# DixianZhu/deBWT

Hardware: AMD Instinct MI355X
Metric: Gbp/sec BWT build (30 Gbp synthetic DNA); bit-exact vs CPU ref; 1/2/4/8-GPU (higher is better)
Workload: dtype u64

## Files before the change

debwt_amd/_lib.py:

```python
import ctypes
import os
import subprocess

_HERE = os.path.dirname(os.path.abspath(__file__))
LIB_PATH = os.environ.get("DEBWT_HIP_LIB", os.path.join(_HERE, "libdebwt_hip.so"))
_lib = None


class DebwtConfig(ctypes.Structure):
    _fields_ = [("k", ctypes.c_int), ("device", ctypes.c_int), ("sort_algo", ctypes.c_int),
                ("reserved", ctypes.c_int)]


class DebwtPackedText(ctypes.Structure):
    _fields_ = [("words", ctypes.POINTER(ctypes.c_uint64)), ("nwords", ctypes.c_uint64), ("n", ctypes.c_uint64),
                ("sep", ctypes.POINTER(ctypes.c_uint64)), ("nrec", ctypes.c_uint64),
                ("seconds_read", ctypes.c_double), ("seconds_pack", ctypes.c_double)]


class DebwtStats(ctypes.Structure):
    _fields_ = ([(n, ctypes.c_uint64) for n in (
        "n", "nrec", "red_capacity", "blue_capacity", "blue_bound_num", "case3num", "sp_len",
        "special_branch_num", "n_main", "distinct_keys", "blue_large_blocks", "blue_max_block")] +
        [(n, ctypes.c_float) for n in (
# ... 231 lines not shown


class DebwtFmMapStats(ctypes.Structure):
    _fields_ = ([(n, ctypes.c_uint64) for n in ("reads", "mapped", "mems", "seeds", "candidates", "jobs", "batches")] +
                [(n, ctypes.c_float) for n in ("ms_mems", "ms_locate", "ms_candidates", "ms_extend", "ms_wall")])

    def as_dict(self):
        return {n: getattr(self, n) for n, _ in self._fields_}


class DebwtMultiStats(ctypes.Structure):
    _fields_ = [("n", ctypes.c_uint64), ("nrec", ctypes.c_uint64), ("ngpus", ctypes.c_uint32), ("rounds", ctypes.c_uint32),
                ("key_bytes_in", ctypes.c_uint64), ("blue_bytes_in", ctypes.c_uint64), ("ms_build", ctypes.c_float),
                ("key_mode", ctypes.c_uint32), ("exchange_backend", ctypes.c_uint32)]

    def as_dict(self):
        return {n: getattr(self, n) for n, _ in self._fields_}


SYMBOLS = [
    "debwt_create", "debwt_destroy", "debwt_strerror", "debwt_last_error", "debwt_load_text",
    "debwt_load_ascii", "debwt_kmer_sort_rle", "debwt_classify", "debwt_sp_generate", "debwt_blue_sort",
    "debwt_bwt_assemble", "debwt_build", "debwt_fetch_bwt", "debwt_bwt_device_ptr", "debwt_get_stats",
    "debwt_fetch_array", "debwt_kmer_count_sorted", "debwt_radix_sort_u64", "debwt_radix_sort_u64_range", "debwt_radix_pair_passes", "debwt_radix_bucket_passes", "debwt_verify_inverse",
    "debwt_shard_begin", "debwt_shard_histogram", "debwt_shard_set_range", "debwt_shard_classify_local",
    "debwt_shard_facts_export", "debwt_shard_classify_global", "debwt_shard_info", "debwt_shard_fetch",
    "debwt_shard_partition_keys", "debwt_shard_plan", "debwt_shard_ranges", "debwt_shard_sort_begin",
    "debwt_shard_sort_range", "debwt_shard_sort_end", "debwt_concat_rows", "debwt_shard_export", "debwt_census_words", "debwt_shard_sp_flags", "debwt_shard_sp_emit",
    "debwt_shard_sp_import", "debwt_shard_blue_route", "debwt_shard_blue_place", "debwt_set_range_cap", "debwt_pack_fasta", "debwt_free_packed", "debwt_load_fasta", "debwt_pack_fasta_opts", "debwt_load_fasta_opts", "debwt_fasta_text_bound", "debwt_host_release_hold", "debwt_special_digest", "debwt_bwt_census", "debwt_fetch_rows", "debwt_verify_device", "debwt_multi_create", "debwt_multi_destroy", "debwt_multi_last_error",
    "debwt_multi_load_text", "debwt_multi_load_fasta", "debwt_multi_build", "debwt_multi_fetch_bwt", "debwt_multi_get_stats",
    "debwt_multi_verify", "debwt_multi_shard", "debwt_pinned_alloc", "debwt_pinned_free", "debwt_shard_key_mode",
    "debwt_multi_set_key_mode", "debwt_special_compare", "debwt_build_to_host", "debwt_multi_set_exchange", "debwt_reserve",
    "debwt_multi_set_serial", "debwt_multi_get_shard_report", "debwt_multi_step_name", "debwt_get_config",
    "debwt_dump_reference_files", "debwt_shard_scratch",
    "debwt_fm_create", "debwt_fm_open", "debwt_fm_last_error", "debwt_fm_info_get", "debwt_fm_samples",
    "debwt_fm_record_starts", "debwt_fm_count", "debwt_fm_locate", "debwt_fm_destroy",
    "debwt_fm_search", "debwt_fm_search_stats_get", "debwt_fm_mems", "debwt_fm_mems_stats_get",
    "debwt_fm_attach_text", "debwt_fm_extend", "debwt_fm_extend_stats_get", "debwt_fm_cluster_seeds",
    "debwt_fm_map_defaults", "debwt_fm_map", "debwt_fm_map_stats_get",
    "debwt_fm_chain_seeds", "debwt_fm_extend_chain", "debwt_fm_chain_defaults", "debwt_fm_map_chained",
    "debwt_fm_align_window", "debwt_fm_insert_bounds", "debwt_fm_pair_select", "debwt_fm_pair_defaults",
    "debwt_fm_map_pairs", "debwt_fm_pair_stats_get",
    "debwt_fm_overlaps", "debwt_fm_overlaps_stats_get", "debwt_fm_overlap_longest",
    "debwt_fm_overlaps_mm", "debwt_fm_overlaps_mm_stats_get",
    "debwt_fm_extract", "debwt_fm_extract_stats_get", "debwt_fm_restore_text", "debwt_fm_text_fetch",
    "debwt_fm_kmer_counts", "debwt_fm_kmer_stats_get", "debwt_fm_weak_trials", "debwt_fm_correct_defaults",
    "debwt_fm_correct", "debwt_fm_correct_stats_get",
# ... 39 lines not shown
        fn = getattr(L, name)
        fn.restype = ctypes.c_int
        fn.argtypes = [vp]
    L.debwt_fetch_bwt.restype = ctypes.c_int
    L.debwt_fetch_bwt.argtypes = [vp, u64p, u64p, u64p]
    L.debwt_reserve.restype = ctypes.c_int
    L.debwt_reserve.argtypes = [vp, ctypes.c_uint64, ctypes.c_uint64, ctypes.c_double, ctypes.c_uint]
    L.debwt_build_to_host.restype = ctypes.c_int
    L.debwt_build_to_host.argtypes = [vp, u64p, u64p, u64p]
    L.debwt_bwt_device_ptr.restype = ctypes.c_int
    L.debwt_bwt_device_ptr.argtypes = [vp, ctypes.POINTER(vp)]
    L.debwt_get_stats.restype = ctypes.c_int
    L.debwt_get_stats.argtypes = [vp, ctypes.POINTER(DebwtStats)]
    L.debwt_fetch_array.restype = ctypes.c_int
    L.debwt_fetch_array.argtypes = [vp, ctypes.c_int, vp, ctypes.c_uint64, u64p]
    L.debwt_kmer_count_sorted.restype = ctypes.c_int
    L.debwt_kmer_count_sorted.argtypes = [vp, u64p, u64p, ctypes.c_uint64, u64p]
    L.debwt_radix_sort_u64.restype = ctypes.c_int
    L.debwt_radix_sort_u64.argtypes = [vp, vp, vp, ctypes.c_uint64, ctypes.c_int, ctypes.POINTER(ctypes.c_float)]
    L.debwt_radix_pair_passes.restype = ctypes.c_uint64
    L.debwt_radix_pair_passes.argtypes = []
    L.debwt_radix_bucket_passes.restype = ctypes.c_uint64
    L.debwt_radix_bucket_passes.argtypes = []
    L.debwt_radix_sort_u64_range.restype = ctypes.c_int
    L.debwt_radix_sort_u64_range.argtypes = [vp, vp, vp, ctypes.c_uint64, ctypes.c_int, ctypes.c_uint64, ctypes.c_uint64,
                                             ctypes.POINTER(ctypes.c_float)]
    L.debwt_verify_inverse.restype = ctypes.c_int
    L.debwt_verify_inverse.argtypes = [u64p, ctypes.c_uint64, u64p, ctypes.c_uint64, ctypes.c_uint64,
                                       ctypes.POINTER(ctypes.c_uint8)]
    L.debwt_shard_begin.restype = ctypes.c_int
    L.debwt_shard_begin.argtypes = [vp, ctypes.c_int, ctypes.c_int]
    L.debwt_shard_histogram.restype = ctypes.c_int
    L.debwt_shard_histogram.argtypes = [vp, u64p]
    L.debwt_shard_set_range.restype = ctypes.c_int
    L.debwt_shard_set_range.argtypes = [vp, ctypes.c_uint32, ctypes.c_uint32, ctypes.c_uint64, ctypes.c_uint64]
    L.debwt_shard_classify_local.restype = ctypes.c_int
    L.debwt_shard_classify_local.argtypes = [vp, u64p, u64p, u64p]
    L.debwt_shard_facts_export.restype = ctypes.c_int
    L.debwt_shard_facts_export.argtypes = [vp, vp, ctypes.c_uint64]
    L.debwt_shard_classify_global.restype = ctypes.c_int
    L.debwt_shard_classify_global.argtypes = [vp, vp, ctypes.c_uint64, ctypes.c_uint64, ctypes.c_uint64]
    u8p, u32p = ctypes.POINTER(ctypes.c_uint8), ctypes.POINTER(ctypes.c_uint32)
    L.debwt_shard_partition_keys.restype = ctypes.c_int
    L.debwt_shard_partition_keys.argtypes = [vp, u8p, vp, ctypes.c_uint64, u64p]
    L.debwt_shard_plan.restype = ctypes.c_int
    L.debwt_shard_plan.argtypes = [vp, u64p, ctypes.c_uint32, ctypes.c_uint32, ctypes.c_uint64, ctypes.c_int,
# ... 214 lines not shown
```

debwt_amd/csrc/debwt_hip.hip:

```cpp
#include "../../include/debwt_hip.h"

#include <hip/hip_runtime.h>

#include <algorithm>
#include <new>
#include <chrono>
#include <cmath>
#include <cstdio>
#include <cstring>
#include <atomic>
#include <string>
#include <thread>
#include <tuple>
#include <vector>

#include "radix_sort.h"
#include "special_host.h"
#include "fasta_host.h"
#include "gz_parallel.h"
#include "stage_kernels.h"
#include "special_kernels.h"
#include "verify_kernels.h"
#include "fm_kernels.h"
#include "fm_search_kernels.h"
// ... 2336 lines not shown
    KmerInfoF f{sorted, Mk, k, c->dk.as<u64>(), c->dstart.as<u32>()};
    if ((rc = cp_count(c, f, Mk, cp_area(c, 0), 0))) return rc;
    if ((rc = cp_emit(c, f, Mk, cp_area(c, 0)))) return rc;
    if ((rc = sync_check(c))) return rc;
    u64 D = c->h_scalars[0];
    *distinct = D;
    u64 ncopy = std::min<u64>(D, capacity);
    if (kmers && ncopy) HIPCHK(c, hipMemcpy(kmers, c->dk.p, ncopy * 8, hipMemcpyDeviceToHost));
    if (counts && ncopy) {
        std::vector<u32> first(D);
        HIPCHK(c, hipMemcpy(first.data(), c->dstart.p, D * 4, hipMemcpyDeviceToHost));
        for (u64 i = 0; i < ncopy; i++) counts[i] = (i + 1 < D ? first[i + 1] : (u32)Mk) - first[i];
    }
    return DEBWT_OK;
}

extern "C" int debwt_radix_sort_u64(debwt_ctx *c, uint64_t *d_keys, uint64_t *d_tmp, uint64_t count, int key_bits,
                                    float *ms_per_pass) {
    return debwt_radix_sort_u64_range(c, d_keys, d_tmp, count, key_bits, 0, 0, ms_per_pass);
}

extern "C" uint64_t debwt_radix_pair_passes(void) { return radix_pair_passes(); }
extern "C" uint64_t debwt_radix_bucket_passes(void) { return radix_bucket_passes(); }

__global__ void k_keys_outside(const u64 *__restrict__ keys, u64 n, u64 lo, u64 hi, u32 *__restrict__ flag) {
    bool bad = false;
    for (u64 i = (u64)blockIdx.x * blockDim.x + threadIdx.x; i < n; i += (u64)gridDim.x * blockDim.x) bad |= keys[i] < lo || keys[i] > hi;
    if (bad) *flag = 1u;
}

extern "C" int debwt_radix_sort_u64_range(debwt_ctx *c, uint64_t *d_keys, uint64_t *d_tmp, uint64_t count, int key_bits,
                                          uint64_t key_lo, uint64_t key_hi, float *ms_per_pass) {
    if (!c || !d_keys || !d_tmp || key_bits < 1 || key_bits > 64) return DEBWT_EINVAL;
    if (key_hi && key_hi <= key_lo) return DEBWT_EINVAL;
    if (count >= 0xFFFFFFF0ull) return DEBWT_ERANGE;
    HIPCHK(c, hipSetDevice(c->cfg.device));
    ENSURE(c, c->rs_skew, (count / 2048 + 2) * 4);
    ENSURE(c, c->rs_over, radix_over_bytes(count));
    const u64 range[2] = {key_lo, key_hi};
    const u64 *rg = key_lo || key_hi ? range : nullptr;
    if (rg) {
        const u64 top = key_bits >= 64 ? ~0ull : (1ull << key_bits) - 1ull;
        u32 outside = 0;
        HIPCHK(c, hipMemsetAsync(c->rs_over.p, 0, 4, c->stream));
        k_keys_outside<<<(u32)std::min<u64>(2048, (count + 255) / 256), 256, 0, c->stream>>>((const u64 *)d_keys, count, key_lo, key_hi ? key_hi - 1 : top,
                                                                                            c->rs_over.as<u32>());
// ... 3626 lines not shown
```

debwt_amd/csrc/radix_sort.h:

```cpp
#pragma once
#include "common.h"

#define RS_BLOCK 256
#ifndef RS_ITEMS
#define RS_ITEMS 16
#endif
#define RS_TILE (RS_BLOCK * RS_ITEMS)
#ifndef RS_MAXCHUNKS
#define RS_MAXCHUNKS 16384
#endif
#define RS_MINCHUNKS 2048
#ifndef RS_CHUNK_TILES
#define RS_CHUNK_TILES 64
#endif
#define RS_RADIX 256

struct RadixWorkspace {
    u32 *counts;
    u32 *over;
    u32 *h_over;
    u32 over_cap;
    u32 *skew_list;
    u32 *pair;
    size_t pair_cap;
};

size_t radix_pair_bytes(u64 n, int lo_bit, int hi_bit, bool aux, const u64 *range);
size_t radix_pair_bytes_u64(u64 n, int key_bits, const u64 *range, bool heavy = false);
u64 radix_pair_passes();

struct RadixSplit { bool hybrid, bucket; int T, pshift, hbm_shift; };
RadixSplit radix_split(u64 n, int key_bits, int algo, const u64 *range, bool heavy);
u64 radix_bucket_passes();
#define RS_BUCKET_HEAVY (1u << 20)

struct TextKeySrc {
    const u64 *text;
    const u64 *sepbits;
    u64 n;
    int K;
    u64 key_lo, key_hi;
    u64 pos0;
    const u32 *pre_counts;
    const u8 *bin_tab;
    int bin_shift;
};

#define RS_MAX_RANGES 16
size_t radix_text_hist_stride();
hipError_t radix_text_hist_ranges(hipStream_t stream, const TextKeySrc &text, const u8 *range_of_bin, int key_bits,
                                  const int *shift, int nranges, u32 *counts);

struct RsDigit {
    int shift; u32 mask;
    int mode;
    const u8 *tab; int tshift;
// ... 30 lines not shown
```

debwt_amd/csrc/radix_sort.hip:

```cpp
#include "radix_sort.h"

#include <algorithm>
#include <atomic>
#include <cstddef>
#include <utility>
#include <cstdio>
#include <cstdlib>
#include <vector>


template <int FIXED0>
__device__ __forceinline__ u32 rs_digit(const RsDigit &g, u64 k) {
    if (FIXED0 == 2) return __builtin_amdgcn_ubfe((u32)(k >> 32), (u32)g.shift - 32u, (u32)__popc(g.mask));
    if (FIXED0 || g.mode == 0) {
        const u32 lo = (u32)k, hi = (u32)(k >> 32);
        const bool up = g.shift >= 32;
        return __builtin_amdgcn_alignbit(up ? 0u : hi, up ? hi : lo, (u32)g.shift & 31u) & g.mask;
    }
    if (g.mode == 1) return g.tab[(k >> g.tshift) & 4095u];
    u32 q = (u32)(k >> g.tshift), lo = 0, hi = g.nb;
    if (hi <= 16u) {
        for (u32 i = 1; i < hi; i++) lo += g.bounds[i] <= q ? 1u : 0u;
        return lo;
    }
// ... 950 lines not shown
    const u64 p = keys[x - 1] >> pshift;
    for (u64 base = x; base < x + reach; base += 64) {
        u64 i = base + lane;
        bool diff = i >= n || (keys[i] >> pshift) != p;
        u64 mk = __ballot(diff);
        if (mk) return base + (u64)__ffsll((long long)mk) - 1;
    }
    u64 lo = x + reach, hi = n;
    while (lo < hi) {
        u64 mid = (lo + hi) >> 1;
        if ((keys[mid] >> pshift) <= p) lo = mid + 1; else hi = mid;
    }
    return lo;
}

#define RL_PAD(x) ((x) + ((x) >> 4))

__device__ __forceinline__ void rl_cex(u64 &a, u64 &b, bool up) {
    bool sw = (a > b) == up;
    u64 lo = sw ? b : a, hi = sw ? a : b;
    a = lo; b = hi;
}

__device__ __forceinline__ void rl_sort16(u64 (&k)[16]) {
#define RL_CE(a, b) rl_cex(k[a], k[b], true)
    RL_CE(0, 13); RL_CE(1, 12); RL_CE(2, 15); RL_CE(3, 14); RL_CE(4, 8); RL_CE(5, 6); RL_CE(7, 11); RL_CE(9, 10);
    RL_CE(0, 5); RL_CE(1, 7); RL_CE(2, 9); RL_CE(3, 4); RL_CE(6, 13); RL_CE(8, 14); RL_CE(10, 15); RL_CE(11, 12);
    RL_CE(0, 1); RL_CE(2, 3); RL_CE(4, 5); RL_CE(6, 8); RL_CE(7, 9); RL_CE(10, 11); RL_CE(12, 13); RL_CE(14, 15);
    RL_CE(0, 2); RL_CE(1, 3); RL_CE(4, 10); RL_CE(5, 11); RL_CE(6, 7); RL_CE(8, 9); RL_CE(12, 14); RL_CE(13, 15);
    RL_CE(1, 2); RL_CE(3, 12); RL_CE(4, 6); RL_CE(5, 7); RL_CE(8, 10); RL_CE(9, 11); RL_CE(13, 14);
    RL_CE(1, 4); RL_CE(2, 6); RL_CE(5, 8); RL_CE(7, 10); RL_CE(9, 13); RL_CE(11, 14);
    RL_CE(2, 4); RL_CE(3, 6); RL_CE(9, 12); RL_CE(11, 13);
    RL_CE(3, 5); RL_CE(6, 8); RL_CE(7, 9); RL_CE(10, 12);
    RL_CE(3, 4); RL_CE(5, 6); RL_CE(7, 8); RL_CE(9, 10); RL_CE(11, 12);
    RL_CE(6, 7); RL_CE(8, 9);
#undef RL_CE
}

template <int LG>
__device__ __forceinline__ void rl_network(u64 (&k)[16], u64 *A, const u32 tid, const bool active) {
    constexpr int KPT = 16;
#pragma unroll
    for (int lk = 1; lk <= LG; lk++) {
        const u32 kk = 1u << lk;
#pragma unroll
        for (int lj = lk - 1; lj >= 0; lj--) {
            if (lj < 4) {
                const int jj = 1 << lj;
// ... 19 lines not shown
                const u32 dt = 1u << (lj - 4);
                if (active) {
#pragma unroll
                    for (int r = 0; r < KPT; r++) A[RL_PAD(tid * KPT + r)] = k[r];
                }
                __syncthreads();
                const bool lower = (tid & dt) == 0;
                if (active) {
#pragma unroll
                    for (int r = 0; r < KPT; r++) {
                        u64 pk = A[RL_PAD((tid ^ dt) * KPT + r)];
                        bool up = ((tid * KPT + r) & kk) == 0;
                        bool take_min = lower == up;
                        bool pless = pk < k[r];
                        k[r] = (take_min == pless) ? pk : k[r];
                    }
                }
                __syncthreads();
            }
        }
    }
}

template <int NT>
__global__ __launch_bounds__(NT) void rs_local_kernel(u64 *__restrict__ keys, u64 n, int pshift,
                                                       u32 *__restrict__ over, u32 over_cap, u8 *__restrict__ mark) {
    constexpr int KPT = 16;
    constexpr u32 CAP = NT * KPT;
    constexpr u32 H = NT == 64 ? RLW_H : RL_H;
    constexpr int LOGN = NT == 64 ? 10 : 12;
    static_assert(NT == 64 || NT == 256, "wave or 4-wave workgroup");
    __shared__ u64 A[CAP + CAP / 16];
    __shared__ u64 sb[2];
    const u32 tid = threadIdx.x;
    if (NT == 256 && !mark[blockIdx.x]) return;
    const u64 x0 = (u64)blockIdx.x * H, x1 = x0 + H;
    if (NT == 64) {
        u64 v0 = x0 == 0 ? 0 : rl_boundary(keys, n, x0, pshift, CAP - H);
        u64 v1 = x1 >= n ? n : rl_boundary(keys, n, x1, pshift, CAP - H);
        if (tid == 0) { sb[0] = v0; sb[1] = v1; }
    } else {
        if ((tid >> 6) == 0) { u64 v = x0 == 0 ? 0 : rl_boundary(keys, n, x0, pshift, CAP - H); if (tid == 0) sb[0] = v; }
        if ((tid >> 6) == 1) { u64 v = x1 >= n ? n : rl_boundary(keys, n, x1, pshift, CAP - H); if (tid == 64) sb[1] = v; }
    }
    __syncthreads();
    const u64 s = sb[0], e = sb[1];
    if (s >= e) return;
// ... 10 lines not shown
            u32 idx = atomicAdd(&over[0], 1u);
            if (idx < over_cap) {
                u64 *list = reinterpret_cast<u64 *>(over + 4);
                list[2 * idx] = s; list[2 * idx + 1] = cnt64;
            }
        }
        return;
    }
    const u32 cnt = (u32)cnt64;
    for (u32 i = tid; i < CAP; i += NT) A[RL_PAD(i)] = i < cnt ? keys[s + i] : ~0ull;
    __syncthreads();
    u64 k[KPT];
#pragma unroll
    for (int r = 0; r < KPT; r++) k[r] = A[RL_PAD(tid * KPT + r)];
    {
        u32 bad = 0;
#pragma unroll
        for (int r = 0; r + 1 < KPT; r++) bad |= k[r] > k[r + 1] ? 1u : 0u;
        if (tid + 1 < NT) bad |= k[KPT - 1] > A[RL_PAD((tid + 1) * KPT)] ? 1u : 0u;
        if (NT == 64 ? (__ballot(bad != 0) == 0ull) : !__syncthreads_or((int)bad)) return;
    }
    __syncthreads();
    bool sorted = false;
    if (NT == 64) {
        rl_sort16(k);
        for (int round = 0; round < RL_MAX_ROUNDS; round++) {
            u64 nxt = __shfl_down(k[0], 1, 64);
            bool ok = tid == 63 || k[KPT - 1] <= nxt;
            if (__ballot(!ok) == 0ull) { sorted = true; break; }
            const bool odd = round & 1;
            const bool lower = ((tid ^ (u32)odd) & 1u) == 0;
            const int partner = lower ? (int)tid + 1 : (int)tid - 1;
            const bool active = partner >= 0 && partner < 64;
            const int src = active ? partner : (int)tid;
            u64 t[KPT];
#pragma unroll
            for (int r = 0; r < KPT; r++) t[r] = __shfl(k[KPT - 1 - r], src, 64);
            if (active) {
#pragma unroll
                for (int r = 0; r < KPT; r++) {
                    bool pless = t[r] < k[r];
                    k[r] = (lower == pless) ? t[r] : k[r];
                }
#pragma unroll
                for (int lj = 3; lj >= 0; lj--) {
                    const int jj = 1 << lj;
#pragma unroll
                    for (int r = 0; r < KPT; r++)
                        if ((r & jj) == 0) rl_cex(k[r], k[r | jj], true);
                }
            }
        }
        if (!sorted) {
            u64 nxt = __shfl_down(k[0], 1, 64);
            bool ok = tid == 63 || k[KPT - 1] <= nxt;
            sorted = __ballot(!ok) == 0ull;
        }
    }
    if (!sorted) {
        if (NT == 256 && cnt <= CAP / 2) rl_network<LOGN - 1>(k, A, tid, tid < NT / 2);
        else rl_network<LOGN>(k, A, tid, true);
    }
#pragma unroll
    for (int r = 0; r < KPT; r++) A[RL_PAD(tid * KPT + r)] = k[r];
    __syncthreads();
    for (u32 i = tid; i < cnt; i += NT) keys[s + i] = A[RL_PAD(i)];
}


__device__ __forceinline__ void rlw_sort(u64 (&k)[16], const u32 lane) {
    constexpr int KPT = 16;
    bool sorted;
    {
        u32 bad = 0;
#pragma unroll
        for (int r = 0; r + 1 < KPT; r++) bad |= k[r] > k[r + 1] ? 1u : 0u;
        const u64 nxt = __shfl_down(k[0], 1, 64);
        if (lane < 63) bad |= k[KPT - 1] > nxt ? 1u : 0u;
        sorted = __ballot(bad != 0) == 0ull;
    }
    if (!sorted) {
        rl_sort16(k);
        for (int round = 0; round < RL_MAX_ROUNDS; round++) {
            const u64 nxt = __shfl_down(k[0], 1, 64);
            const bool ok = lane == 63 || k[KPT - 1] <= nxt;
            if (__ballot(!ok) == 0ull) { sorted = true; break; }
            const bool odd = round & 1;
            const bool lower = ((lane ^ (u32)odd) & 1u) == 0;
            const int partner = lower ? (int)lane + 1 : (int)lane - 1;
            const bool active = partner >= 0 && partner < 64;
            const int src = active ? partner : (int)lane;
            u64 t[KPT];
#pragma unroll
            for (int r = 0; r < KPT; r++) t[r] = __shfl(k[KPT - 1 - r], src, 64);
            if (active) {
#pragma unroll
                for (int r = 0; r < KPT; r++) {
                    const bool pless = t[r] < k[r];
                    k[r] = (lower == pless) ? t[r] : k[r];
                }
#pragma unroll
                for (int lj = 3; lj >= 0; lj--) {
                    const int jj = 1 << lj;
#pragma unroll
                    for (int r = 0; r < KPT; r++)
                        if ((r & jj) == 0) rl_cex(k[r], k[r | jj], true);
                }
            }
        }
        if (!sorted) {
            const u64 nxt = __shfl_down(k[0], 1, 64);
            const bool ok = lane == 63 || k[KPT - 1] <= nxt;
            sorted = __ballot(!ok) == 0ull;
        }
    }
    if (!sorted) {
#pragma unroll
        for (int lk = 1; lk <= 10; lk++) {
            const u32 kk = 1u << lk;
#pragma unroll
            for (int lj = lk - 1; lj >= 0; lj--) {
                if (lj < 4) {
                    const int jj = 1 << lj;
#pragma unroll
                    for (int r = 0; r < KPT; r++)
                        if ((r & jj) == 0) rl_cex(k[r], k[r | jj], ((lane * KPT + r) & kk) == 0);
                } else {
                    const int dl = 1 << (lj - 4);
                    const bool lower = (lane & dl) == 0;
#pragma unroll
                    for (int r = 0; r < KPT; r++) {
                        const u64 pk = __shfl_xor(k[r], dl, 64);
                        const bool up = ((lane * KPT + r) & kk) == 0;
                        const bool take_min = lower == up;
                        const bool pless = pk < k[r];
                        k[r] = (take_min == pless) ? pk : k[r];
                    }
                }
            }
        }
    }
}

#define RLT_STAGED 0x80000000u
#ifndef RLT_STAGE_RATIO
#define RLT_STAGE_RATIO 2u
#endif
#ifndef RLW_WINDOW
#define RLW_WINDOW 1
#endif
__global__ __launch_bounds__(64) void rs_local_count_kernel(u64 *__restrict__ keys, u64 n, int pshift,
                                                            u8 *__restrict__ mark, u64 *__restrict__ bnd,
                                                            u32 *__restrict__ unfit, u32 *__restrict__ nunfit,
                                                            u32 *__restrict__ tcnt, u8 *__restrict__ mchar,
                                                            u64 *__restrict__ stg, int drop_sorted) {
    constexpr int KPT = 16;
    constexpr u32 CAP = RLW_CAP;
    const u32 lane = threadIdx.x;
    const u64 x0 = (u64)blockIdx.x * RLW_H, x1 = x0 + RLW_H;
#if RLW_WINDOW
    constexpr u32 REACH = RLW_CAP - RLW_H, NR = 18, WN = NR * 64;
    static_assert(RLW_H + REACH + 1 <= WN && REACH + RLW_CAP <= WN, "the window holds every boundary slot and every fit tile");
    __shared__ u64 A[WN + WN / 16];
    {
        u64 g[NR];
#pragma unroll
        for (u32 r = 0; r < NR; r++) {
            const u64 p1 = x0 + r * 64u + lane;
            g[r] = (p1 >= 1 && p1 - 1 < n) ? keys[p1 - 1] : ~0ull;
        }
#pragma unroll
        for (u32 r = 0; r < NR; r++) A[RL_PAD(r * 64u + lane)] = g[r];
    }
// ... 26 lines not shown
        if (lane == 0) {
            unfit[atomicAdd(nunfit, 1u)] = blockIdx.x;
            if ((e - x0) / RLW_H >= RLU_LONG) unfit[gridDim.x - 1u - atomicAdd(nunfit + 2, 1u)] = blockIdx.x;
        }
        return;
    }
    const u32 cnt = (u32)(e - s);
    u64 k[KPT];
#if RLW_WINDOW
    if (s - x0 + 1 + cnt <= WN) {
        const u32 off = (u32)(s - x0) + 1u;
#pragma unroll
        for (int r = 0; r < KPT; r++) k[r] = lane * KPT + r < cnt ? A[RL_PAD(off + lane * KPT + r)] : ~0ull;
    } else {
        for (u32 i = lane; i < CAP; i += 64) A[RL_PAD(i)] = i < cnt ? keys[s + i] : ~0ull;
#pragma unroll
        for (int r = 0; r < KPT; r++) k[r] = A[RL_PAD(lane * KPT + r)];
    }
#else
    for (u32 i = lane; i < CAP; i += 64) A[RL_PAD(i)] = i < cnt ? keys[s + i] : ~0ull;
#pragma unroll
    for (int r = 0; r < KPT; r++) k[r] = A[RL_PAD(lane * KPT + r)];
#endif
    rlw_sort(k, lane);
#pragma unroll
    for (int r = 0; r < KPT; r++) A[RL_PAD(lane * KPT + r)] = k[r];
    const u64 before = __shfl_up(k[KPT - 1], 1, 64);
    u32 hm = 0;
#pragma unroll
    for (int r = 0; r < KPT; r++) {
        const u64 p = r ? k[r - 1] : before;
        hm |= ((lane * KPT + r < cnt && ((lane == 0 && r == 0) || k[r] != p)) ? 1u : 0u) << r;
    }
    const u32 cl = (u32)__popc(hm), incl = wave_scan_incl(cl);
    const u32 c = (u32)__shfl((int)incl, 63, 64);
    const bool staged = stg != nullptr && RLT_STAGE_RATIO * c <= cnt;
    if (lane == 0) tcnt[blockIdx.x] = c | (staged ? RLT_STAGED : 0u);
    if (staged) {
        u64 *kd = stg + s;
        unsigned short *id = reinterpret_cast<unsigned short *>(stg + s + c);
        u32 o = incl - cl;
#pragma unroll
        for (int r = 0; r < KPT; r++)
            if ((hm >> r) & 1u) { kd[o] = k[r]; id[o] = (unsigned short)(lane * KPT + r); o++; }
    }
    if (lane * KPT < cnt) {
        u8 *dst = mchar + s + lane * KPT;
// ... 758 lines not shown
        else if (shift >= 32) rs_scatter_kernel<0, 0, 1><<<nchunks, SC_NT, 0, stream>>>(src, none, dst, n, chunk, dg, ws.counts, digit_tot, nchunks, ctab);
        else rs_scatter_kernel<0, 0, 0><<<nchunks, SC_NT, 0, stream>>>(src, none, dst, n, chunk, dg, ws.counts, digit_tot, nchunks, ctab);
        if (ev) { (void)hipEventRecord(pass_events[2 * ev_idx + 1], stream); ev_idx++; if (npairs) *npairs = ev_idx; }
        derived = pp.nv != 0;
        if (derived) {
            rs_pair_bounds_kernel<<<(nchunks + 1 + 255) / 256, 256, 0, stream>>>(ws.counts, digit_tot, nchunks, pp.rows, n, chunk, nchunks, pair_tab);
            rs_pair_derive_kernel<<<nchunks, RS_RADIX, 0, stream>>>(pair_J, pair_tab, pp.nv, pp.vbase, ws.counts, nchunks);
            rs_pair_launched.fetch_add(1, std::memory_order_relaxed);
        }
        if (final_dst) { src = dst; dst = (npasses - (p + 2)) % 2 == 0 ? final_dst : (src == a ? third : a); }
        else if (third) { src = dst; dst = p + 2 == npasses ? a : (src == b ? third : b); }
        else { u64 *t = src; src = dst; dst = t; }
    }
    return src;
}

size_t radix_text_hist_stride() { return (size_t)RS_RADIX * RS_MAXCHUNKS; }

static int rs_bucket_mode() {
    const char *e = getenv("DEBWT_BUCKET_PASS");
    return !e || !*e ? -1 : (atoi(e) != 0 ? 1 : 0);
}

RadixSplit radix_split(u64 n, int key_bits, int algo, const u64 *range, bool heavy) {
    algo &= 15;
    if (key_bits > 64) key_bits = 64;
    const int mode = rs_bucket_mode();
    int T = 0;
    while ((n >> (8 * T)) > RS_BUCKET_TARGET && T < 4) T++;
    if (mode == 1 && T < 2) T = 2;
    RadixSplit sp{false, false, 0, 0, 0};
    if (algo != 3 || T == 0 || key_bits - 8 * T < 1) return sp;
    sp.hybrid = true;
    sp.T = T;
    sp.pshift = key_bits - 8 * T;
    const bool ranged = range && (range[0] || range[1]);
    sp.bucket = mode == 1 ? T >= 2 : (mode != 0 && T == 4 && ranged && !heavy);
    sp.hbm_shift = sp.bucket ? sp.pshift + 8 : sp.pshift;
    return sp;
}

static std::atomic<u64> rs_bucket_launched{0};
u64 radix_bucket_passes() { return rs_bucket_launched.load(std::memory_order_relaxed); }

hipError_t radix_text_hist_ranges(hipStream_t stream, const TextKeySrc &text, const u8 *range_of_bin, int key_bits,
                                  const int *shift, int nranges, u32 *counts) {
    if (nranges < 1 || nranges > RS_MAX_RANGES) return hipErrorInvalidValue;
    u32 nchunks; u64 chunk;
    rs_plan(text.n, &nchunks, &chunk);
    RangeShifts sh{};
    for (int i = 0; i < nranges; i++) sh.s[i] = shift[i];
    TextKeySrc all = text;
    all.key_lo = 0; all.key_hi = 0; all.pre_counts = nullptr;
    bool words = (text.pos0 & 31ull) == 0 && text.K >= 16;
    for (int i = 0; i < nranges; i++) words = words && shift[i] >= 34 - (64 - 2 * text.K) && shift[i] + (64 - 2 * text.K) - 34 <= 24;
    if (words)
        rs_hist_ranges_words_kernel<<<nchunks, RS_BLOCK, 0, stream>>>(all, chunk, range_of_bin, sh, nranges, counts,
                                                                       (u64)radix_text_hist_stride(), nchunks);
    else
        rs_hist_ranges_kernel<<<nchunks, RS_BLOCK, 0, stream>>>(all, chunk, range_of_bin, key_bits - 12, sh, nranges, counts,
                                                                 (u64)radix_text_hist_stride(), nchunks);
    return hipGetLastError();
}

u64 *radix_sort_bits(hipStream_t stream, u64 *a, u64 *b, u64 n, int lo_bit, int hi_bit, const RadixWorkspace &ws,
                     hipError_t *err, int strip_last, bool *stripped, u64 *third) {
// ... 29 lines not shown
    const bool aux = (algo & 16) != 0;
    const bool net_only = (algo & 32) != 0;
    (void)net_only;
    algo &= 15;
    if (key_bits > 64) key_bits = 64;
    if (!text && (n < (rs_bucket_mode() == 1 ? 1u : 2u) || key_bits <= 0)) return a;
    const u64 text_range[2] = {text ? text->key_lo : 0ull, text ? text->key_hi : 0ull};
    if (!key_range && text) key_range = text_range;
    const RadixSplit sp = radix_split(n, key_bits, algo, key_range, heavy);
    if (!sp.hybrid || !ws.over || !ws.h_over) {
        u64 *r = rs_lsd(stream, a, b, n, 0, key_bits, ws, pass_events, max_pairs, npairs, text, aux, 0, nullptr, nullptr, key_range);
        *err = hipGetLastError();
        return r;
    }
    const int pshift = sp.pshift;
    u64 *src = rs_lsd(stream, a, b, n, sp.hbm_shift, key_bits, ws, pass_events, max_pairs, npairs, text, aux, 0, nullptr, nullptr, key_range);
    u64 *other = src == a ? b : a;
    if (sp.bucket && n > 0) {
        const u32 nbt = (u32)((n + RB_H - 1) / RB_H);
        rs_bucket_digit_kernel<<<nbt, RB_NT, 0, stream>>>(src, other, n, sp.hbm_shift, pshift);
        rs_bucket_launched.fetch_add(1, std::memory_order_relaxed);
        u64 *t = src; src = other; other = t;
    }
    (void)hipMemsetAsync(ws.over, 0, 16, stream);
    u32 ntiles = (u32)((n + RL_H - 1) / RL_H), nwtiles = (u32)((n + RLW_H - 1) / RLW_H);
    u8 *mark = reinterpret_cast<u8 *>(ws.skew_list);
    (void)hipMemsetAsync(mark, 0, ntiles + 1, stream);
    u32 *rle_ctr = nullptr, *rle_tcnt = nullptr, *rle_unfit = nullptr, *rle_tex = nullptr, *rle_bsum = nullptr, *rle_boff = nullptr;
    u64 *rle_bnd = nullptr;
    if (sink) {
        const size_t nw = rle_nw(n);
        rle_ctr = static_cast<u32 *>(sink->ws);
        rle_bnd = reinterpret_cast<u64 *>(rle_ctr + 4);
        rle_tcnt = reinterpret_cast<u32 *>(rle_bnd + nw);
        rle_unfit = rle_tcnt + nw;
        rle_tex = rle_unfit + nw;
        rle_bsum = rle_tex + nw;
        rle_boff = rle_bsum + rle_nb(n);
        (void)hipMemsetAsync(rle_ctr, 0, 16, stream);
        rs_local_count_kernel<<<nwtiles, 64, 0, stream>>>(src, n, pshift, mark, rle_bnd, rle_unfit, rle_ctr, rle_tcnt, sink->mchar,
                                                          sink->no_staging ? nullptr : other, sink->drop_sorted ? 1 : 0);
        const u32 ugrid = nwtiles < 16384u ? nwtiles : 16384u;
#if RLU_CLASSIFY
        u64 *const stg = sink->no_staging ? nullptr : other;
        rs_local_unfit_kernel<8><<<ugrid, 256, 0, stream>>>(src, n, rle_bnd, nwtiles, rle_unfit, rle_ctr, ws.over, ws.over_cap,
                                                            net_only ? 0u : RLU_GAP_MAX, rle_tcnt, sink->mchar, stg, sink->drop_sorted ? 1 : 0);
        rs_local_unfit_kernel<16><<<ugrid < 4096u ? ugrid : 4096u, 256, 0, stream>>>(src, n, rle_bnd, nwtiles, rle_unfit, rle_ctr, ws.over,
                                                                                      ws.over_cap, net_only ? 0u : RLU_GAP_MAX,
                                                                                      rle_tcnt, sink->mchar, stg, sink->drop_sorted ? 1 : 0);
#endif
        rs_local_unfit_net_kernel<<<ugrid, 256, 0, stream>>>(src, n, rle_bnd, nwtiles, rle_unfit, rle_ctr, ws.over, ws.over_cap);
    } else {
        rs_local_kernel<64><<<nwtiles, 64, 0, stream>>>(src, n, pshift, ws.over, ws.over_cap, mark);
        rs_local_kernel<256><<<ntiles, 256, 0, stream>>>(src, n, pshift, ws.over, ws.over_cap, mark);
    }
    (void)hipMemcpyAsync(ws.h_over, ws.over, 16, hipMemcpyDeviceToHost, stream);
    if ((*err = hipStreamSynchronize(stream)) != hipSuccess) return src;
    u32 nover = ws.h_over[0];
    bool staging_lost = false;
    if (nover) {
        bool whole = nover > ws.over_cap;
        u64 total = 0;
        std::vector<u64> offs, hlist;
        if (!whole) {
            hlist.resize(2 * (size_t)nover);
            (void)hipMemcpyAsync(hlist.data(), ws.over + 4, 16 * (size_t)nover, hipMemcpyDeviceToHost, stream);
            if ((*err = hipStreamSynchronize(stream)) != hipSuccess) return src;
            const u64 *list = hlist.data();
            std::vector<std::pair<u64, u64>> rg(nover);
            for (u32 i = 0; i < nover; i++) rg[i] = {list[2 * i], list[2 * i + 1]};
            std::sort(rg.begin(), rg.end());
            offs.resize(3 * (size_t)nover);
            for (u32 i = 0; i < nover; i++) {
                offs[i] = total; total += rg[i].second;
                offs[nover + 2 * i] = rg[i].first; offs[nover + 2 * i + 1] = rg[i].second;
            }
// ... 109 lines not shown
```

include/debwt_hip.h:

```cpp
#ifndef DEBWT_HIP_H
#define DEBWT_HIP_H
#include <stddef.h>
#include <stdint.h>
#ifdef __cplusplus
extern "C" {
#endif

#define DEBWT_OK 0
#define DEBWT_EINVAL (-1)
#define DEBWT_ENOMEM (-2)
#define DEBWT_EDEVICE (-3)
#define DEBWT_ESTATE (-4)
#define DEBWT_ERANGE (-5)
#define DEBWT_EINTERNAL (-6)
#define DEBWT_EIO (-7)

typedef struct debwt_ctx debwt_ctx;

typedef struct {
    int k;
    int device;
    int sort_algo;
    int reserved;
} debwt_config;
// ... 152 lines not shown
    DEBWT_ARR_SP_SYMBOLS,
    DEBWT_ARR_BLUE,
    DEBWT_ARR_BLUE_BOUND,
    DEBWT_ARR_CASE3_BOUND,
    DEBWT_ARR_ROW_SYMBOLS
} debwt_array;
int debwt_fetch_array(debwt_ctx *ctx, debwt_array which, void *dst, uint64_t capacity, uint64_t *count);

#define DEBWT_DUMP_KMERINFO 1
#define DEBWT_DUMP_BLOCKS 2
#define DEBWT_DUMP_SP 3
int debwt_dump_reference_files(debwt_ctx *ctx, const char *dir, int stage);


int debwt_kmer_count_sorted(debwt_ctx *ctx, uint64_t *kmers, uint64_t *counts, uint64_t capacity,
                            uint64_t *distinct);

int debwt_radix_sort_u64(debwt_ctx *ctx, uint64_t *d_keys, uint64_t *d_tmp, uint64_t count, int key_bits,
                         float *ms_per_pass);
int debwt_radix_sort_u64_range(debwt_ctx *ctx, uint64_t *d_keys, uint64_t *d_tmp, uint64_t count, int key_bits,
                               uint64_t key_lo, uint64_t key_hi, float *ms_per_pass);
uint64_t debwt_radix_pair_passes(void);
uint64_t debwt_radix_bucket_passes(void);

int debwt_special_digest(const uint64_t *packed, uint64_t n, const uint64_t *sep, uint64_t nrec, int k, uint64_t digest[4]);

int debwt_special_compare(debwt_ctx *ctx, uint64_t mismatch[6]);

int debwt_verify_inverse(const uint64_t *bwt, uint64_t n, const uint64_t *hash_rows, uint64_t nrec,
                         uint64_t dollar_row, uint8_t *sym_out);

typedef struct {
    uint64_t segments, steps, mismatches, broken_links, search_failures, search_steps;
    float ms_index, ms_search, ms_walk;
    int ok;
} debwt_verify_report;
int debwt_verify_device(debwt_ctx *ctx, const uint64_t *d_words, const uint64_t *hash_rows, uint64_t dollar_row,
                        uint64_t segments, debwt_verify_report *report);
int debwt_multi_verify(debwt_multi *m, debwt_verify_report *report);

typedef struct debwt_fm debwt_fm;
typedef struct {
    uint64_t n, nrec, sa_sample, samples, device_bytes;
    float ms_rank, ms_samples;
    uint64_t census[4];
} debwt_fm_info;
// ... 257 lines not shown
```

Measured before the change: 23.78.

## Finish local radix tiles sorting only low 32 bits with DPP lane exchanges

When the remaining prefix shift is at most 32 bits, the wave-local sort in the local-finish kernels compares full keys but moves only the low 32-bit halves. Because the high halves are already equal within a tile, it exchanges neighbour values with DPP row shifts instead of 64-bit shuffles. The aim is to halve register traffic and cross-lane data movement in the odd-even merge rounds. It also adds an env-forced prefix digit count and a counter of low finishes, and relies on the assumption that high bits are uniform within each tile.

```diff
diff --git a/debwt_amd/_lib.py b/debwt_amd/_lib.py
--- a/debwt_amd/_lib.py
+++ b/debwt_amd/_lib.py
@@ -277,7 +277,7 @@
     "debwt_create", "debwt_destroy", "debwt_strerror", "debwt_last_error", "debwt_load_text",
     "debwt_load_ascii", "debwt_kmer_sort_rle", "debwt_classify", "debwt_sp_generate", "debwt_blue_sort",
     "debwt_bwt_assemble", "debwt_build", "debwt_fetch_bwt", "debwt_bwt_device_ptr", "debwt_get_stats",
-    "debwt_fetch_array", "debwt_kmer_count_sorted", "debwt_radix_sort_u64", "debwt_radix_sort_u64_range", "debwt_radix_pair_passes", "debwt_radix_bucket_passes", "debwt_verify_inverse",
+    "debwt_fetch_array", "debwt_kmer_count_sorted", "debwt_radix_sort_u64", "debwt_radix_sort_u64_range", "debwt_radix_pair_passes", "debwt_radix_bucket_passes", "debwt_radix_low_finishes", "debwt_verify_inverse",
     "debwt_shard_begin", "debwt_shard_histogram", "debwt_shard_set_range", "debwt_shard_classify_local",
     "debwt_shard_facts_export", "debwt_shard_classify_global", "debwt_shard_info", "debwt_shard_fetch",
     "debwt_shard_partition_keys", "debwt_shard_plan", "debwt_shard_ranges", "debwt_shard_sort_begin",
@@ -363,6 +363,8 @@
     L.debwt_radix_pair_passes.argtypes = []
     L.debwt_radix_bucket_passes.restype = ctypes.c_uint64
     L.debwt_radix_bucket_passes.argtypes = []
+    L.debwt_radix_low_finishes.restype = ctypes.c_uint64
+    L.debwt_radix_low_finishes.argtypes = []
     L.debwt_radix_sort_u64_range.restype = ctypes.c_int
     L.debwt_radix_sort_u64_range.argtypes = [vp, vp, vp, ctypes.c_uint64, ctypes.c_int, ctypes.c_uint64, ctypes.c_uint64,
                                              ctypes.POINTER(ctypes.c_float)]
diff --git a/debwt_amd/csrc/debwt_hip.hip b/debwt_amd/csrc/debwt_hip.hip
--- a/debwt_amd/csrc/debwt_hip.hip
+++ b/debwt_amd/csrc/debwt_hip.hip
@@ -2382,6 +2382,7 @@
 
 extern "C" uint64_t debwt_radix_pair_passes(void) { return radix_pair_passes(); }
 extern "C" uint64_t debwt_radix_bucket_passes(void) { return radix_bucket_passes(); }
+extern "C" uint64_t debwt_radix_low_finishes(void) { return radix_low_finishes(); }
 
 __global__ void k_keys_outside(const u64 *__restrict__ keys, u64 n, u64 lo, u64 hi, u32 *__restrict__ flag) {
     bool bad = false;
diff --git a/debwt_amd/csrc/radix_sort.h b/debwt_amd/csrc/radix_sort.h
--- a/debwt_amd/csrc/radix_sort.h
+++ b/debwt_amd/csrc/radix_sort.h
@@ -32,6 +32,7 @@
 struct RadixSplit { bool hybrid, bucket; int T, pshift, hbm_shift; };
 RadixSplit radix_split(u64 n, int key_bits, int algo, const u64 *range, bool heavy);
 u64 radix_bucket_passes();
+u64 radix_low_finishes();
 #define RS_BUCKET_HEAVY (1u << 20)
 
 struct TextKeySrc {
diff --git a/debwt_amd/csrc/radix_sort.hip b/debwt_amd/csrc/radix_sort.hip
--- a/debwt_amd/csrc/radix_sort.hip
+++ b/debwt_amd/csrc/radix_sort.hip
@@ -996,8 +996,16 @@
     a = lo; b = hi;
 }
 
+__device__ __forceinline__ void rl_cex_low(u64 &a, u64 &b) {
+    const bool sw = __builtin_amdgcn_inverse_ballot_w64(__builtin_amdgcn_ballot_w64(a > b));
+    const u32 al = (u32)a, bl = (u32)b;
+    a = (a & 0xffffffff00000000ull) | (sw ? bl : al);
+    b = (b & 0xffffffff00000000ull) | (sw ? al : bl);
+}
+
+template <bool LOW = false>
 __device__ __forceinline__ void rl_sort16(u64 (&k)[16]) {
-#define RL_CE(a, b) rl_cex(k[a], k[b], true)
+#define RL_CE(a, b) do { if (LOW) rl_cex_low(k[a], k[b]); else rl_cex(k[a], k[b], true); } while (0)
     RL_CE(0, 13); RL_CE(1, 12); RL_CE(2, 15); RL_CE(3, 14); RL_CE(4, 8); RL_CE(5, 6); RL_CE(7, 11); RL_CE(9, 10);
     RL_CE(0, 5); RL_CE(1, 7); RL_CE(2, 9); RL_CE(3, 4); RL_CE(6, 13); RL_CE(8, 14); RL_CE(10, 15); RL_CE(11, 12);
     RL_CE(0, 1); RL_CE(2, 3); RL_CE(4, 5); RL_CE(6, 8); RL_CE(7, 9); RL_CE(10, 11); RL_CE(12, 13); RL_CE(14, 15);
@@ -1063,7 +1071,108 @@
     }
 }
 
-template <int NT>
+#ifndef RLW_DPP
+#define RLW_DPP 1
+#endif
+
+template <bool ODD>
+__device__ __forceinline__ u32 rlw_partner(const u32 old, const u32 v, const u32 lane) {
+    if (RLW_DPP > (ODD ? 1 : 0)) {
+        if (!ODD) return (u32)__builtin_amdgcn_update_dpp((int)old, (int)v, 0xB1, 0xf, 0xf, false);
+        const u32 up = (u32)__builtin_amdgcn_update_dpp((int)old, (int)v, 0x130, 0xf, 0xf, false);
+        const u32 dn = (u32)__builtin_amdgcn_update_dpp((int)old, (int)v, 0x138, 0xf, 0xf, false);
+        return (lane & 1u) ? up : dn;
+    }
+    const int p = ODD ? ((lane & 1u) ? (int)lane + 1 : (int)lane - 1) : (int)(lane ^ 1u);
+    return (u32)__shfl((int)v, p < 0 || p > 63 ? (int)lane : p, 64);
+}
+
+template <bool ODD>
+__device__ __forceinline__ void rlw_round_low(u64 (&k)[16], u64 (&pt)[16], const u32 lane) {
+    constexpr int KPT = 16;
+    const bool lower = ((lane ^ (ODD ? 1u : 0u)) & 1u) == 0;
+    const bool active = !ODD || (lane > 0 && lane < 63);
+#pragma unroll
+    for (int r = 0; r < KPT; r++) pt[r] = (pt[r] & 0xffffffff00000000ull) | rlw_partner<ODD>((u32)pt[r], (u32)k[KPT - 1 - r], lane);
+    if (active) {
+#pragma unroll
+        for (int r = 0; r < KPT; r++) {
+            const bool pless = pt[r] < k[r];
+            k[r] = (k[r] & 0xffffffff00000000ull) | ((lower == pless) ? (u32)pt[r] : (u32)k[r]);
+        }
+#pragma unroll
+        for (int lj = 3; lj >= 0; lj--) {
+            const int jj = 1 << lj;
+#pragma unroll
+            for (int r = 0; r < KPT; r++)
+                if ((r & jj) == 0) rl_cex_low(k[r], k[r | jj]);
+        }
+    }
+}
+
+__device__ __forceinline__ bool rlw_in_order(const u64 (&k)[16], const u32 lane) {
+    const u64 nxt = __shfl_down(k[0], 1, 64);
+    const bool ok = lane == 63 || k[15] <= nxt;
+    return __ballot(!ok) == 0ull;
+}
+
+template <bool LOW>
+__device__ __forceinline__ bool rlw_rounds(u64 (&k)[16], const u32 lane) {
+    constexpr int KPT = 16;
+    bool sorted = false;
+    rl_sort16<LOW>(k);
+    if (LOW) {
+        sorted = rlw_in_order(k, lane);
+        if (!sorted) {
+            u64 pt[2][KPT];
+#pragma unroll
+            for (int r = 0; r < KPT; r++) {
+                pt[0][r] = (u64)rlw_partner<false>(0u, (u32)(k[KPT - 1 - r] >> 32), lane) << 32;
+                pt[1][r] = (u64)rlw_partner<true>(0u, (u32)(k[KPT - 1 - r] >> 32), lane) << 32;
+            }
+            for (int round = 0; round < RL_MAX_ROUNDS; round += 2) {
+                rlw_round_low<false>(k, pt[0], lane);
+                if (rlw_in_order(k, lane)) { sorted = true; break; }
+                if (round + 1 < RL_MAX_ROUNDS) {
+                    rlw_round_low<true>(k, pt[1], lane);
+                    if (rlw_in_order(k, lane)) { sorted = true; break; }
+                }
+            }
+        }
+        return sorted;
+    }
+    for (int round = 0; round < RL_MAX_ROUNDS; round++) {
+        const u64 nxt = __shfl_down(k[0], 1, 64);
+        const bool ok = lane == 63 || k[KPT - 1] <= nxt;
+        if (__ballot(!ok) == 0ull) { sorted = true; break; }
+        const bool odd = round & 1;
+        const bool lower = ((lane ^ (u32)odd) & 1u) == 0;
+        const int partner = lower ? (int)lane + 1 : (int)lane - 1;
+        const bool active = partner >= 0 && partner < 64;
+        const int src = active ? partner : (int)lane;
+        u64 t[KPT];
+#pragma unroll
+        for (int r = 0; r < KPT; r++) t[r] = __shfl(k[KPT - 1 - r], src, 64);
+        if (active) {
+#pragma unroll
+            for (int r = 0; r < KPT; r++) {
+                const bool pless = t[r] < k[r];
+                k[r] = (lower == pless) ? t[r] : k[r];
+            }
+#pragma unroll
+            for (int lj = 3; lj >= 0; lj--) {
+                const int jj = 1 << lj;
+#pragma unroll
+                for (int r = 0; r < KPT; r++)
+                    if ((r & jj) == 0) rl_cex(k[r], k[r | jj], true);
+            }
+        }
+    }
+    if (!sorted) sorted = rlw_in_order(k, lane);
+    return sorted;
+}
+
+template <int NT, bool LOW = false>
 __global__ __launch_bounds__(NT) void rs_local_kernel(u64 *__restrict__ keys, u64 n, int pshift,
                                                        u32 *__restrict__ over, u32 over_cap, u8 *__restrict__ mark) {
     constexpr int KPT = 16;
@@ -1120,41 +1229,7 @@
     }
     __syncthreads();
     bool sorted = false;
-    if (NT == 64) {
-        rl_sort16(k);
-        for (int round = 0; round < RL_MAX_ROUNDS; round++) {
-            u64 nxt = __shfl_down(k[0], 1, 64);
-            bool ok = tid == 63 || k[KPT - 1] <= nxt;
-            if (__ballot(!ok) == 0ull) { sorted = true; break; }
-            const bool odd = round & 1;
-            const bool lower = ((tid ^ (u32)odd) & 1u) == 0;
-            const int partner = lower ? (int)tid + 1 : (int)tid - 1;
-            const bool active = partner >= 0 && partner < 64;
-            const int src = active ? partner : (int)tid;
-            u64 t[KPT];
-#pragma unroll
-            for (int r = 0; r < KPT; r++) t[r] = __shfl(k[KPT - 1 - r], src, 64);
-            if (active) {
-#pragma unroll
-                for (int r = 0; r < KPT; r++) {
-                    bool pless = t[r] < k[r];
-                    k[r] = (lower == pless) ? t[r] : k[r];
-                }
-#pragma unroll
-                for (int lj = 3; lj >= 0; lj--) {
-                    const int jj = 1 << lj;
-#pragma unroll
-                    for (int r = 0; r < KPT; r++)
-                        if ((r & jj) == 0) rl_cex(k[r], k[r | jj], true);
-                }
-            }
-        }
-        if (!sorted) {
-            u64 nxt = __shfl_down(k[0], 1, 64);
-            bool ok = tid == 63 || k[KPT - 1] <= nxt;
-            sorted = __ballot(!ok) == 0ull;
-        }
-    }
+    if (NT == 64) sorted = rlw_rounds<LOW>(k, tid);
     if (!sorted) {
         if (NT == 256 && cnt <= CAP / 2) rl_network<LOGN - 1>(k, A, tid, tid < NT / 2);
         else rl_network<LOGN>(k, A, tid, true);
@@ -1166,6 +1241,7 @@
 }
 
 
+template <bool LOW>
 __device__ __forceinline__ void rlw_sort(u64 (&k)[16], const u32 lane) {
     constexpr int KPT = 16;
     bool sorted;
@@ -1177,41 +1253,7 @@
         if (lane < 63) bad |= k[KPT - 1] > nxt ? 1u : 0u;
         sorted = __ballot(bad != 0) == 0ull;
     }
-    if (!sorted) {
-        rl_sort16(k);
-        for (int round = 0; round < RL_MAX_ROUNDS; round++) {
-            const u64 nxt = __shfl_down(k[0], 1, 64);
-            const bool ok = lane == 63 || k[KPT - 1] <= nxt;
-            if (__ballot(!ok) == 0ull) { sorted = true; break; }
-            const bool odd = round & 1;
-            const bool lower = ((lane ^ (u32)odd) & 1u) == 0;
-            const int partner = lower ? (int)lane + 1 : (int)lane - 1;
-            const bool active = partner >= 0 && partner < 64;
-            const int src = active ? partner : (int)lane;
-            u64 t[KPT];
-#pragma unroll
-            for (int r = 0; r < KPT; r++) t[r] = __shfl(k[KPT - 1 - r], src, 64);
-            if (active) {
-#pragma unroll
-                for (int r = 0; r < KPT; r++) {
-                    const bool pless = t[r] < k[r];
-                    k[r] = (lower == pless) ? t[r] : k[r];
-                }
-#pragma unroll
-                for (int lj = 3; lj >= 0; lj--) {
-                    const int jj = 1 << lj;
-#pragma unroll
-                    for (int r = 0; r < KPT; r++)
-                        if ((r & jj) == 0) rl_cex(k[r], k[r | jj], true);
-                }
-            }
-        }
-        if (!sorted) {
-            const u64 nxt = __shfl_down(k[0], 1, 64);
-            const bool ok = lane == 63 || k[KPT - 1] <= nxt;
-            sorted = __ballot(!ok) == 0ull;
-        }
-    }
+    if (!sorted) sorted = rlw_rounds<LOW>(k, lane);
     if (!sorted) {
 #pragma unroll
         for (int lk = 1; lk <= 10; lk++) {
@@ -1247,6 +1289,7 @@
 #ifndef RLW_WINDOW
 #define RLW_WINDOW 1
 #endif
+template <bool LOW>
 __global__ __launch_bounds__(64) void rs_local_count_kernel(u64 *__restrict__ keys, u64 n, int pshift,
                                                             u8 *__restrict__ mark, u64 *__restrict__ bnd,
                                                             u32 *__restrict__ unfit, u32 *__restrict__ nunfit,
@@ -1319,7 +1362,7 @@
 #pragma unroll
     for (int r = 0; r < KPT; r++) k[r] = A[RL_PAD(lane * KPT + r)];
 #endif
-    rlw_sort(k, lane);
+    rlw_sort<LOW>(k, lane);
 #pragma unroll
     for (int r = 0; r < KPT; r++) A[RL_PAD(lane * KPT + r)] = k[r];
     const u64 before = __shfl_up(k[KPT - 1], 1, 64);
@@ -2124,6 +2167,16 @@
     return !e || !*e ? -1 : (atoi(e) != 0 ? 1 : 0);
 }
 
+static int rs_forced_digits() {
+    const char *e = getenv("DEBWT_PREFIX_DIGITS");
+    const int t = e && *e ? atoi(e) : 0;
+    return t >= 1 && t <= 4 ? t : 0;
+}
+static bool rs_finish_low() {
+    const char *e = getenv("DEBWT_FINISH_LOW");
+    return !e || !*e || atoi(e) != 0;
+}
+
 RadixSplit radix_split(u64 n, int key_bits, int algo, const u64 *range, bool heavy) {
     algo &= 15;
     if (key_bits > 64) key_bits = 64;
@@ -2131,6 +2184,7 @@
     int T = 0;
     while ((n >> (8 * T)) > RS_BUCKET_TARGET && T < 4) T++;
     if (mode == 1 && T < 2) T = 2;
+    if (rs_forced_digits()) T = rs_forced_digits();
     RadixSplit sp{false, false, 0, 0, 0};
     if (algo != 3 || T == 0 || key_bits - 8 * T < 1) return sp;
     sp.hybrid = true;
@@ -2144,6 +2198,8 @@
 
 static std::atomic<u64> rs_bucket_launched{0};
 u64 radix_bucket_passes() { return rs_bucket_launched.load(std::memory_order_relaxed); }
+static std::atomic<u64> rs_low_finishes{0};
+u64 radix_low_finishes() { return rs_low_finishes.load(std::memory_order_relaxed); }
 
 hipError_t radix_text_hist_ranges(hipStream_t stream, const TextKeySrc &text, const u8 *range_of_bin, int key_bits,
                                   const int *shift, int nranges, u32 *counts) {
@@ -2219,6 +2275,8 @@
         rs_bucket_launched.fetch_add(1, std::memory_order_relaxed);
         u64 *t = src; src = other; other = t;
     }
+    const bool low = pshift <= 32 && rs_finish_low();
+    if (low) rs_low_finishes.fetch_add(1, std::memory_order_relaxed);
     (void)hipMemsetAsync(ws.over, 0, 16, stream);
     u32 ntiles = (u32)((n + RL_H - 1) / RL_H), nwtiles = (u32)((n + RLW_H - 1) / RLW_H);
     u8 *mark = reinterpret_cast<u8 *>(ws.skew_list);
@@ -2235,8 +2293,12 @@
         rle_bsum = rle_tex + nw;
         rle_boff = rle_bsum + rle_nb(n);
         (void)hipMemsetAsync(rle_ctr, 0, 16, stream);
-        rs_local_count_kernel<<<nwtiles, 64, 0, stream>>>(src, n, pshift, mark, rle_bnd, rle_unfit, rle_ctr, rle_tcnt, sink->mchar,
-                                                          sink->no_staging ? nullptr : other, sink->drop_sorted ? 1 : 0);
+        if (low)
+            rs_local_count_kernel<true><<<nwtiles, 64, 0, stream>>>(src, n, pshift, mark, rle_bnd, rle_unfit, rle_ctr, rle_tcnt, sink->mchar,
+                                                                    sink->no_staging ? nullptr : other, sink->drop_sorted ? 1 : 0);
+        else
+            rs_local_count_kernel<false><<<nwtiles, 64, 0, stream>>>(src, n, pshift, mark, rle_bnd, rle_unfit, rle_ctr, rle_tcnt, sink->mchar,
+                                                                     sink->no_staging ? nullptr : other, sink->drop_sorted ? 1 : 0);
         const u32 ugrid = nwtiles < 16384u ? nwtiles : 16384u;
 #if RLU_CLASSIFY
         u64 *const stg = sink->no_staging ? nullptr : other;
@@ -2248,7 +2310,8 @@
 #endif
         rs_local_unfit_net_kernel<<<ugrid, 256, 0, stream>>>(src, n, rle_bnd, nwtiles, rle_unfit, rle_ctr, ws.over, ws.over_cap);
     } else {
-        rs_local_kernel<64><<<nwtiles, 64, 0, stream>>>(src, n, pshift, ws.over, ws.over_cap, mark);
+        if (low) rs_local_kernel<64, true><<<nwtiles, 64, 0, stream>>>(src, n, pshift, ws.over, ws.over_cap, mark);
+        else rs_local_kernel<64><<<nwtiles, 64, 0, stream>>>(src, n, pshift, ws.over, ws.over_cap, mark);
         rs_local_kernel<256><<<ntiles, 256, 0, stream>>>(src, n, pshift, ws.over, ws.over_cap, mark);
     }
     (void)hipMemcpyAsync(ws.h_over, ws.over, 16, hipMemcpyDeviceToHost, stream);
diff --git a/include/debwt_hip.h b/include/debwt_hip.h
--- a/include/debwt_hip.h
+++ b/include/debwt_hip.h
@@ -198,6 +198,7 @@
                                uint64_t key_lo, uint64_t key_hi, float *ms_per_pass);
 uint64_t debwt_radix_pair_passes(void);
 uint64_t debwt_radix_bucket_passes(void);
+uint64_t debwt_radix_low_finishes(void);
 
 int debwt_special_digest(const uint64_t *packed, uint64_t n, const uint64_t *sep, uint64_t nrec, int k, uint64_t digest[4]);
 
```

Result: faster. 24.31, median of 6 (+2.2%).
